# cfdeinza/reinforcement-learning-rendezvous

Measured on AMD Instinct MI355X. Metric: env steps/sec, higher is better.
Workload: dtype f64

## Files before the change

### reinforcement_learning_rendezvous_amd/csrc/rdv_rollout.h

```cpp
#pragma once

namespace rdv {

constexpr int kRollEnvs = 256;
constexpr int kRollEnvWaves = kRollEnvs / kWave;
constexpr int kRollActorWaves = kRollEnvs / kPolWaveEnvs;
constexpr int kRollBlock = (kRollEnvWaves + kRollActorWaves) * kWave;
constexpr int kRollLdsFloats = kPolFloats + kRollEnvs * RDV_ACT_DIM + kRollEnvs * RDV_OBS_DIM + kRollEnvs * RDV_ACT_DIM +
                               kRollEnvWaves * kStatWords * 2 + 2 * kRollEnvs;
constexpr int kRollLdsFixed = kRollLdsFloats * 4 + kSlotObsVecs * kRollEnvs * 16 + kRollEnvWaves * kRollEnvs * 2;
template <typename ST> constexpr int roll_lds_bytes() { return kRollLdsFixed + kChunks * kRollEnvs * 4 * (int)sizeof(ST); }
static_assert(roll_lds_bytes<double>() <= 160 * 1024, "the rollout workgroup must fit the CU's 160 KiB of LDS");
static_assert(kRollEnvs == kGroupEnvs, "refill_pass_lds is written for 256-env workgroups");


struct RolloutArgs {
  void* ws;
  uint64_t* stats;
  float* obs;
  float* actions;
  float* reward;
  uint8_t* done;
  float* log_prob;
  float* last_obs;
// ... 27 lines not shown
  using V = typename Vec4<ST>::type;
  extern __shared__ __attribute__((aligned(16))) float lds[];
  float* w = lds;
  float* act_raw = w + kPolFloats;
  float* obs_cur = act_raw + kRollEnvs * RDV_ACT_DIM;
  float* act_cur = obs_cur + kRollEnvs * RDV_OBS_DIM;
  uint64_t* stat_lds = reinterpret_cast<uint64_t*>(act_cur + kRollEnvs * RDV_ACT_DIM);
  uint32_t* job_kind = reinterpret_cast<uint32_t*>(stat_lds + kRollEnvWaves * kStatWords);
  uint32_t* job_counter = job_kind + kRollEnvs;
  uint32_t* refills_done = reinterpret_cast<uint32_t*>(stat_lds + (kStatWords - 1));
  V* slot_chunks = reinterpret_cast<V*>(job_counter + kRollEnvs);
  float4* slot_obs = reinterpret_cast<float4*>(slot_chunks + kChunks * kRollEnvs);
  const SlotStore<ST> L = lds_slot_store<ST>(slot_chunks, slot_obs, kRollEnvs);
  uint16_t* lists = reinterpret_cast<uint16_t*>(slot_obs + kSlotObsVecs * kRollEnvs);
  const bool resets = A.on_done == RDV_ON_DONE_RESET;
  const DevParams& P = *Pp;
  const int lane = threadIdx.x & (kWave - 1);
  const int wv = threadIdx.x >> 6;
  const bool env_role = wv < kRollEnvWaves;
  const int64_t n = A.n;
  const int64_t block_base = (int64_t)blockIdx.x * kRollEnvs;
  const int T = A.n_steps;

  for (int q = threadIdx.x; q < kPolFloats / 4; q += kRollBlock)
    *reinterpret_cast<float4*>(w + 4 * q) = *reinterpret_cast<const float4*>(W + 4 * q);

  const int slot = (wv & (kRollEnvWaves - 1)) * kWave + lane;
  const int64_t i = block_base + slot;
  const bool active = env_role && i < n;
  Env e;
  e.episode = 0u;
  bool wt_dirty = kGeneral;
  bool slot_dirty = false;
  const SlotStore<ST> H = hbm_slot_store<ST>(A.prep);
  uint64_t* my_stats = stat_lds + (wv & (kRollEnvWaves - 1)) * kStatWords;
  if (env_role) {
    if (lane < kStatWords) my_stats[lane] = (i - lane < n && lane < 12) ? A.stats[(uint64_t)((i - lane) / kWave) * kStatWords + lane] : 0ull;
    __builtin_amdgcn_s_setprio(2);
    float o[RDV_OBS_DIM];
#pragma unroll
    for (int j = 0; j < RDV_OBS_DIM; ++j) o[j] = 0.0f;
    if (active) {
      load_env<ST>(reinterpret_cast<const V*>(A.ws), A.cs, i, e);
      observation(P, e, o);
    }
#pragma unroll
    for (int j = 0; j < RDV_OBS_DIM; ++j) obs_cur[slot * RDV_OBS_DIM + j] = o[j];
    if (resets) {
      uint32_t tag = 0u;
      if (active) { tag = A.prep_tag[i]; slot_copy<ST>(L, slot, H, i); }
      const bool stale = active && tag != e.episode + 1u;
      job_kind[slot] = stale ? JOB_REFILL : JOB_NONE;
      job_counter[slot] = e.episode;
      slot_dirty = stale;
    }
  }
  __syncthreads();

  const int a_wave = wv - kRollEnvWaves;
  const int r0 = a_wave * kPolWaveEnvs;
  const int64_t a_env0 = block_base + r0;
  const int64_t a_rows = env_role ? 0 : ((n - a_env0) < kPolWaveEnvs ? (n - a_env0) : kPolWaveEnvs);
  float* araw = act_raw + (env_role ? 0 : r0) * RDV_ACT_DIM;
  const bool vec_rows = (n & 3) == 0;

  StepArgs SA;
  SA.diag = nullptr;

  if (!env_role) {
   const bool refills = resets && a_wave < kGroupWaves;
   uint16_t* list = lists + (a_wave & (kGroupWaves - 1)) * kRollEnvs;
   auto draw_noise = [&](int t_next, int ln_) {
     if (A.deterministic || a_rows <= 0) return;
     const int er_ = ln_ & 31, eh_ = ln_ >> 5;
     float z[4];
     actor_noise(ln_, A.noise_seed, A.env_id_offset + (uint64_t)(a_env0 + er_), A.noise_counter0 + (uint64_t)t_next, z);
     if (eh_ == 0) {
#pragma unroll
       for (int c = 0; c < 4; ++c) araw[er_ * RDV_ACT_DIM + c] = z[c];
     } else {
       araw[er_ * RDV_ACT_DIM + 4] = z[0]; araw[er_ * RDV_ACT_DIM + 5] = z[1];
     }
     wave_fence();
   };
   draw_noise(0, lane);
#ifdef RDV_STAMPS
   unsigned long long acc_a = 0, acc_r = 0, acc_w1 = 0, acc_w2 = 0;
#endif
   for (int t = 0; t < T; ++t) {
// ... 186 lines not shown
```

### reinforcement_learning_rendezvous_amd/csrc/rdv_slots.h

```cpp
#pragma once

namespace rdv {

constexpr int kSlotObsVecs = 5;
enum : uint32_t { JOB_NONE = 0, JOB_REFILL = 1 };
constexpr uint32_t kFlagsPending = 0xFFFFFFFFu;

template <typename ST>
struct SlotStore {
  typename Vec4<ST>::type* chunks;
  float4* obs;
  int64_t cs, es, ocs, oes;
  static constexpr bool kLive = false;
  __device__ __forceinline__ typename Vec4<ST>::type* chunk(int c, int64_t i) const { return chunks + (c * cs + i * es); }
  __device__ __forceinline__ float4* ovec(int v, int64_t i) const { return obs + (v * ocs + i * oes); }
  __device__ __forceinline__ float* oelem(int j, int64_t i) const { return reinterpret_cast<float*>(ovec(j >> 2, i)) + (j & 3); }
  __device__ __forceinline__ void opad(int64_t i) const { float* p = oelem(16, i); p[1] = 0.0f; p[2] = 0.0f; p[3] = 0.0f; }
};
template <typename ST>
struct LiveStore {
  typename Vec4<ST>::type* ws;
  float* rows;
  int64_t cs, base;
  static constexpr bool kLive = true;
  __device__ __forceinline__ typename Vec4<ST>::type* chunk(int c, int64_t s) const { return ws + (c * cs + base + s); }
  __device__ __forceinline__ float* oelem(int j, int64_t s) const { return rows + (s * RDV_OBS_DIM + j); }
  __device__ __forceinline__ void opad(int64_t) const {}
};
template <typename ST> constexpr int slot_record_bytes() { return sizeof(ST) == 4 ? 192 : 320; }
template <typename ST>
__device__ __forceinline__ SlotStore<ST> hbm_slot_store(void* prep) {
  using V = typename Vec4<ST>::type;
  SlotStore<ST> S;
  S.chunks = reinterpret_cast<V*>(prep);
  S.obs = reinterpret_cast<float4*>(S.chunks + kChunks);
  S.cs = 1; S.es = slot_record_bytes<ST>() / (int)sizeof(V);
  S.ocs = 1; S.oes = slot_record_bytes<ST>() / 16;
  return S;
}
template <typename ST>
__device__ __forceinline__ SlotStore<ST> lds_slot_store(typename Vec4<ST>::type* chunks, float4* obs, int entries) {
  SlotStore<ST> S;
  S.chunks = chunks; S.obs = obs; S.cs = entries; S.es = 1; S.ocs = entries; S.oes = 1;
  return S;
}

template <typename ST>
__device__ __forceinline__ void slot_store_full(const SlotStore<ST>& S, int64_t i, const Env& ne, const float* o) {
  typename Vec4<ST>::type c[kChunks];
  pack_env<ST>(ne, c);
#pragma unroll
  for (int k = 0; k < kChunks; ++k) *S.chunk(k, i) = c[k];
#pragma unroll
  for (int v = 0; v < 4; ++v) *S.ovec(v, i) = make_float4(o[4 * v], o[4 * v + 1], o[4 * v + 2], o[4 * v + 3]);
  *S.ovec(4, i) = make_float4(o[16], 0.0f, 0.0f, 0.0f);
}

template <typename ST>
struct SlotRaw {
  typename Vec4<ST>::type c[kChunks];
  float4 o[kSlotObsVecs];
};
template <typename ST>
__device__ __forceinline__ void slot_fetch(const SlotStore<ST>& S, int64_t i, SlotRaw<ST>& raw) {
#pragma unroll
  for (int k = 0; k < kChunks; ++k) raw.c[k] = *S.chunk(k, i);
#pragma unroll
  for (int v = 0; v < kSlotObsVecs; ++v) raw.o[v] = *S.ovec(v, i);
}
template <typename ST>
__device__ __forceinline__ void slot_unpack(const DevParams& P, const SlotRaw<ST>& raw, Env& e, float* o) {
  const typename Vec4<ST>::type* c = raw.c;
  e.rc[0] = c[0].x; e.rc[1] = c[0].y; e.rc[2] = c[0].z; e.vc[0] = c[0].w;
  e.vc[1] = c[1].x; e.vc[2] = c[1].y; e.wc[0] = c[1].z; e.wc[1] = c[1].w;
  e.wc[2] = c[2].x; e.bubble = c[2].y; e.sum_dv = c[2].z; e.sum_dw = c[2].w;
  e.qc[0] = c[3].x; e.qc[1] = c[3].y; e.qc[2] = c[3].z; e.qc[3] = c[3].w;
  e.qt[0] = c[4].x; e.qt[1] = c[4].y; e.qt[2] = c[4].z; e.qt[3] = c[4].w;
  e.ep_ret = c[5].x; e.k = (int32_t)s2u(c[5].y); e.flags = s2u(c[5].z); e.episode = s2u(c[5].w);
  e.wt[0] = c[6].x; e.wt[1] = c[6].y; e.wt[2] = c[6].z;
#pragma unroll
  for (int v = 0; v < 4; ++v) { o[4 * v] = raw.o[v].x; o[4 * v + 1] = raw.o[v].y; o[4 * v + 2] = raw.o[v].z; o[4 * v + 3] = raw.o[v].w; }
  o[16] = raw.o[4].x;
  if (e.flags == kFlagsPending) e.flags = reset_flags(P, e);
}

template <typename ST>
__device__ __forceinline__ void slot_copy(const SlotStore<ST>& D, int64_t di, const SlotStore<ST>& S, int64_t si) {
#pragma unroll
  for (int k = 0; k < kChunks; ++k) *D.chunk(k, di) = *S.chunk(k, si);
#pragma unroll
  for (int v = 0; v < kSlotObsVecs; ++v) *D.ovec(v, di) = *S.ovec(v, si);
}

__device__ __forceinline__ const double* tape_row_of(const double* tape, int32_t depth, int64_t n, int64_t i, uint32_t counter) {
  if (depth <= 0) return nullptr;
  uint32_t dep = (uint32_t)depth;
  asm volatile("" : "+s"(dep));
  return tape + ((int64_t)(counter % dep) * n + i) * RDV_STATE_DIM;
}

template <typename ST>
__device__ __forceinline__ void reset_whole(const DevParams& P, Env& ne, float* o, uint64_t seed, uint64_t env_id, uint32_t counter,
                                            const double* tape_row) {
  ne.episode = counter;
  reset_env<ST>(P, ne, seed, env_id, tape_row);
  observation(P, ne, o);
}

template <typename ST>
__device__ __forceinline__ void refill_whole(const StepArgs& A, const DevParams& P, int64_t i, uint32_t counter) {
  Env ne;
  float o[RDV_OBS_DIM];
  reset_whole<ST>(P, ne, o, A.seed, A.env_id_offset + (uint64_t)i, counter, tape_row_of(A.tape, A.tape_depth, A.n, i, counter));
  slot_store_full<ST>(hbm_slot_store<ST>(A.prep), i, ne, o);
  A.prep_tag[i] = counter + 1u;
}

template <typename ST, int kPart, typename Store>
__device__ __forceinline__ void slot_refill_part(const DevParams& P, const Store& S, int64_t i, uint64_t seed, uint64_t env_id,
                                                 uint32_t counter, const double* tape_row) {
  const ST t = ST(0);
  Env ne;
  ne.episode = counter;
  reset_fields<ST, kPart>(P, ne, seed, env_id, tape_row);
  ST* c1 = reinterpret_cast<ST*>(S.chunk(1, i));
  ST* c2 = reinterpret_cast<ST*>(S.chunk(2, i));
  auto O = [&](int j) -> float& { return *S.oelem(j, i); };
  if (kPart == RESET_RC_VC) {
    uint32_t flags = 0u;
    if (reset_flags_needed(P, ne)) {
      flags = kFlagsPending;
      if (Store::kLive) {
        Env full;
        full.episode = counter;
        reset_fields<ST, RESET_ALL>(P, full, seed, env_id, tape_row);
        flags = reset_flags(P, full);
      }
    }
    typename Vec4<ST>::type v0, v5;
    v0.x = (ST)ne.rc[0]; v0.y = (ST)ne.rc[1]; v0.z = (ST)ne.rc[2]; v0.w = (ST)ne.vc[0];
    *S.chunk(0, i) = v0;
    c1[0] = (ST)ne.vc[1]; c1[1] = (ST)ne.vc[2];
    c2[1] = (ST)canon(P.bubble_radius0, t); c2[2] = ST(0); c2[3] = ST(0);
    v5.x = ST(0); v5.y = u2s(0u, t); v5.z = u2s(flags, t); v5.w = u2s(counter + 1u, t);
    *S.chunk(5, i) = v5;
#pragma unroll
    for (int j = 0; j < 3; ++j) {
      const float a = normalized(ne.rc[j], P.obs_lo_r, P.obs_span_r, P.obs_inv_span_r);
      const float b = normalized(ne.vc[j], P.obs_lo_v, P.obs_span_v, P.obs_inv_span_v);
      O(j) = a;
      O(3 + j) = b;
    }
  } else if (kPart == RESET_QC_WC) {
    typename Vec4<ST>::type v3;
    v3.x = (ST)ne.qc[0]; v3.y = (ST)ne.qc[1]; v3.z = (ST)ne.qc[2]; v3.w = (ST)ne.qc[3];
    *S.chunk(3, i) = v3;
    c1[2] = (ST)ne.wc[0]; c1[3] = (ST)ne.wc[1]; c2[0] = (ST)ne.wc[2];
    O(6) = (float)ne.qc[0]; O(7) = (float)ne.qc[1]; O(8) = (float)ne.qc[2]; O(9) = (float)ne.qc[3];
    O(10) = normalized(ne.wc[0], P.obs_lo_w, P.obs_span_w, P.obs_inv_span_w);
    O(11) = normalized(ne.wc[1], P.obs_lo_w, P.obs_span_w, P.obs_inv_span_w);
    O(12) = normalized(ne.wc[2], P.obs_lo_w, P.obs_span_w, P.obs_inv_span_w);
  } else if (kPart == RESET_QT) {
    typename Vec4<ST>::type v4;
    v4.x = (ST)ne.qt[0]; v4.y = (ST)ne.qt[1]; v4.z = (ST)ne.qt[2]; v4.w = (ST)ne.qt[3];
    *S.chunk(4, i) = v4;
    O(13) = (float)ne.qt[0]; O(14) = (float)ne.qt[1]; O(15) = (float)ne.qt[2]; O(16) = (float)ne.qt[3];
    S.opad(i);
  } else {
    typename Vec4<ST>::type v6;
    v6.x = (ST)ne.wt[0]; v6.y = (ST)ne.wt[1]; v6.z = (ST)ne.wt[2]; v6.w = ST(0);
    *S.chunk(6, i) = v6;
  }
}
template <typename ST, typename Store>
__device__ __forceinline__ void slot_refill_role(int role, const DevParams& P, const Store& S, int64_t i, uint64_t seed,
                                                 uint64_t env_id, uint32_t counter, const double* tape_row) {
  if (role == 0) slot_refill_part<ST, RESET_RC_VC>(P, S, i, seed, env_id, counter, tape_row);
  else if (role == 1) slot_refill_part<ST, RESET_QC_WC>(P, S, i, seed, env_id, counter, tape_row);
  else if (role == 2) slot_refill_part<ST, RESET_QT>(P, S, i, seed, env_id, counter, tape_row);
  else slot_refill_part<ST, RESET_WT>(P, S, i, seed, env_id, counter, tape_row);
}

template <int Q>
__device__ __forceinline__ int compact_flags(const bool (&flag)[Q], int lane, uint16_t* list) {
  int total = 0;
#pragma unroll
  for (int q = 0; q < Q; ++q) {
    const unsigned long long m = __ballot(flag[q]);
    if (flag[q]) {
      const int rank = (int)__builtin_amdgcn_mbcnt_hi((uint32_t)(m >> 32), __builtin_amdgcn_mbcnt_lo((uint32_t)m, 0u));
      list[total + rank] = (uint16_t)(q * kWave + lane);
    }
    total += __popcll(m);
  }
  wave_lds_fence();
  return total;
}

constexpr int kGroupEnvs = 256;
constexpr int kGroupWaves = kGroupEnvs / kWave;

template <typename ST, typename Store>
__device__ __forceinline__ void refill_pass_lds(int role, int lane, const DevParams& P, const Store& L, const uint32_t* job_kind,
                                                const uint32_t* job_counter, uint16_t* list, int64_t block_base, int64_t n, uint64_t seed,
                                                uint64_t env_id_offset, const double* tape, int32_t tape_depth) {
// ... 19 lines not shown
```

### reinforcement_learning_rendezvous_amd/csrc/rdv_step.h

```cpp
#pragma once
#include "rdv_kernels.h"
#include "rdv_slots.h"

namespace rdv {

template <typename ST>
__global__ __launch_bounds__(kBlock) void prepare_kernel(const DevParams* __restrict__ Pp, const StepArgs A) {
  using V = typename Vec4<ST>::type;
  const int64_t i = (int64_t)blockIdx.x * kBlock + threadIdx.x;
  if (i >= A.n) return;
  const V c5 = reinterpret_cast<const V*>(A.ws)[5 * A.cs + i];
  refill_whole<ST>(A, *Pp, i, s2u(c5.w));
}

template <typename ST, bool kAll, typename... G>
__global__ __launch_bounds__(kBlock) __attribute__((amdgpu_waves_per_eu(sizeof(ST) == 4 ? RDV_PARTS_WAVES : 3))) void step_kernel_parts(void* ws_hot, const float* actions_hot, const DevParams* __restrict__ Pp, int64_t n_hot,
                                                             uint64_t* stats_hot, float* obs_hot, float* reward_hot, G... tile_group, const StepArgs A_rest) {
  static_assert(sizeof...(G) <= 1, "G is empty or the type of the tile table");
  const StepArgs A = hot_args(A_rest, ws_hot, actions_hot, n_hot, stats_hot, obs_hot, reward_hot);
  using V = typename Vec4<ST>::type;
  __shared__ __attribute__((aligned(16))) float lds[kBlock * RDV_OBS_DIM];
  __shared__ uint32_t job_kind[kBlock];
  __shared__ uint32_t job_counter[kBlock];
  __shared__ uint16_t lists[kGroupWaves * kBlock];
// ... 79 lines not shown
  }
  RDV_STAMP(6);
  if (A.stream_rows) store_obs_rows<true>(A.obs, wave_base, rows, lane, wl);
  else store_obs_rows<false>(A.obs, wave_base, rows, lane, wl);
  RDV_STAMP(7);
  RDV_STAMP_FLUSH((uint64_t)blockIdx.x * (kBlock / kWave) + wave_in_block)
}

constexpr int kSplitEnvs = 256;
constexpr int kSplitBlock = 512;

template <typename ST>
__device__ __forceinline__ void refill_stale_slots(const StepArgs& A, const DevParams& P, int64_t base, int wv, int lane, uint32_t* job_kind,
                                                   uint32_t* job_counter, uint16_t* lists) {
  constexpr int Q = kSplitEnvs / kWave;
  constexpr int kWords = sizeof(typename Vec4<ST>::type) / 4, kWordK = kWords / 4, kWordEpisode = 3 * kWords / 4;
  if (wv < Q) {
    const uint32_t* c5 = reinterpret_cast<const uint32_t*>(reinterpret_cast<const typename Vec4<ST>::type*>(A.ws) + 5 * A.cs);
    const int s = wv * kWave + lane;
    const int64_t ii = base + s;
    const bool ok = ii < A.n;
    const int64_t il = ok ? ii : A.n - 1;
    const uint32_t k = c5[il * kWords + kWordK], episode = c5[il * kWords + kWordEpisode], tag = A.prep_tag[il];
    job_kind[s] = (ok && k == 0u && tag != episode + 1u) ? JOB_REFILL : JOB_NONE;
    job_counter[s] = episode;
  }
  __syncthreads();
  if (wv >= Q) return;
  uint16_t* list = lists + wv * kSplitEnvs;
  bool flag[Q];
#pragma unroll
  for (int q = 0; q < Q; ++q) flag[q] = job_kind[q * kWave + lane] != JOB_NONE;
  const int total = compact_flags<Q>(flag, lane, list);
  const SlotStore<ST> S = hbm_slot_store<ST>(A.prep);
#pragma clang loop unroll(disable)
  for (int j0 = 0; j0 < total; j0 += kWave) {
    const int j = j0 + lane;
    if (j < total) {
      const int s = (int)list[j];
      const uint32_t counter = job_counter[s];
      const int64_t ii = base + s;
      slot_refill_role<ST>(wv, P, S, ii, A.seed, A.env_id_offset + (uint64_t)ii, counter, tape_row_of(A.tape, A.tape_depth, A.n, ii, counter));
      if (wv == 0) A.prep_tag[ii] = counter + 1u;
    }
  }
}

#ifndef RDV_TARGET_SERVICE_PRIO
#define RDV_TARGET_SERVICE_PRIO 3
#endif
#define RDV_REQUEST_RECORDS(rec, recp, mask, saved)                                                                                                  \
  do {                                                                                                                                               \
    _Pragma("unroll") for (int v_ = 0; v_ < 12; ++v_) asm volatile("" : "=v"(rec[v_]));      \
    asm volatile("s_and_saveexec_b64 %[sv], %[m]\n\t"                                                                                                \
                 "global_load_dwordx4 %[r0], %[p], off\n\t"                                                                                          \
                 "global_load_dwordx4 %[r1], %[p], off offset:16\n\t"                                                                                \
                 "global_load_dwordx4 %[r2], %[p], off offset:32\n\t"                                                                                \
                 "global_load_dwordx4 %[r3], %[p], off offset:48\n\t"                                                                                \
                 "global_load_dwordx4 %[r4], %[p], off offset:64\n\t"                                                                                \
                 "global_load_dwordx4 %[r5], %[p], off offset:80\n\t"                                                                                \
                 "global_load_dwordx4 %[r6], %[p], off offset:96\n\t"                                                                                \
                 "global_load_dwordx4 %[r7], %[p], off offset:112\n\t"                                                                               \
                 "global_load_dwordx4 %[r8], %[p], off offset:128\n\t"                                                                               \
                 "global_load_dwordx4 %[r9], %[p], off offset:144\n\t"                                                                               \
                 "global_load_dwordx4 %[r10], %[p], off offset:160\n\t"                                                                              \
                 "global_load_dwordx4 %[r11], %[p], off offset:176\n\t"                                                                              \
                 "s_mov_b64 exec, %[sv]"                                                                                                             \
                 : [r0] "+v"(rec[0]), [r1] "+v"(rec[1]), [r2] "+v"(rec[2]), [r3] "+v"(rec[3]), [r4] "+v"(rec[4]), [r5] "+v"(rec[5]), [r6] "+v"(rec[6]), \
                   [r7] "+v"(rec[7]), [r8] "+v"(rec[8]), [r9] "+v"(rec[9]), [r10] "+v"(rec[10]), [r11] "+v"(rec[11]), [sv] "=&s"(saved)               \
                 : [p] "v"(recp), [m] "s"(mask)                                                                                                      \
                 : "scc");                                                                                                                           \
  } while (0)
template <typename ST, bool kAll, bool kSlots, bool kTarget, bool kObs = false>
__device__ __forceinline__ void split_body(void* ws_hot, const float* actions_hot, const DevParams* Pp, int64_t n_hot, uint64_t* stats_hot, float* obs_hot,
                                           float* reward_hot, const StepArgs& A_rest, float* stage, unsigned long long* fin_mask, float* hand_f, double* hand_d,
                                           float* hand_c = nullptr, unsigned long long* out_mask = nullptr) {
  static_assert(!kTarget || kSlots, "the target form is a form of the slot form");
  static_assert(!kObs || kTarget, "the observation form is a form of the target form");
  constexpr int kS = kTarget ? 1 : 0;
  (void)kS; (void)hand_f; (void)hand_d; (void)hand_c; (void)out_mask;
  const StepArgs A = hot_args(A_rest, ws_hot, actions_hot, n_hot, stats_hot, obs_hot, reward_hot);
  using V = typename Vec4<ST>::type;
  const DevParams& P = *Pp;
  const int lane = threadIdx.x & (kWave - 1);
  const int wv = threadIdx.x >> 6;
  const bool step_role = wv < kSplitEnvs / kWave;
  const int slot_in_block = threadIdx.x & (kSplitEnvs - 1);
  const int64_t n = A.n;
  const int64_t i = (int64_t)blockIdx.x * kSplitEnvs + slot_in_block;
  const int64_t wave_base = i - lane;
  const bool active = i < n;
  const int64_t rows = (n - wave_base) < kWave ? (n - wave_base) : kWave;
  V* ws = reinterpret_cast<V*>(A.ws);
  const bool resets = A.on_done == RDV_ON_DONE_RESET;
  RDV_STAMP_DECL
  RDV_STAMP(0);

  if constexpr (kSlots) {
    static_assert(sizeof(ST) == 4 && kAll, "the slot form is built for fp32 storage without halted envs");
    const unsigned n_step_wgs = (unsigned)((n + kSplitEnvs - 1) / kSplitEnvs);
    const bool refill_role = blockIdx.x >= n_step_wgs;
    const unsigned refill_wg = blockIdx.x - n_step_wgs;
// ... 70 lines not shown
    } else {
      if constexpr (kAll) { advance_all<ST>(P, e, a, r, row_sink, kPack ? packed : nullptr, actions_ready); stepped = active; }
      else stepped = advance<ST, false>(A, P, i, active, e, a, r, row_sink, NoHook(), kPack ? packed : nullptr);
      RDV_STAMP(2);
    }
    bool fin = stepped && r.done;
    bool to_reset = fin && resets;
    const unsigned long long m_reset = __ballot(to_reset);
    if (lane == 0) fin_mask[wv] = m_reset;
    if constexpr (!kObs) {
      halt_if_done<ST>(A, fin, e, kPack ? packed : nullptr);
      if (stepped && !to_reset) { if (kPack) store_chunks<ST, true>(ws, A.cs, i, packed, false); else store_env<ST>(ws, A.cs, i, e, false); }
    }
    RDV_STAMP(3 + kS);
    __syncthreads();
    RDV_STAMP(4 + kS);
    if constexpr (kObs) {
      if ((out_mask[wv] >> lane) & 1ull) { r.done = 1; r.reason = 1; }
      fin = stepped && r.done;
      to_reset = fin && resets;
      halt_if_done<ST>(A, fin, e, packed);
      if (stepped && !to_reset) store_chunks<ST, true>(ws, A.cs, i, packed, false);
    }
    stats_update(slot, slot_pre, lane, stepped, fin, r.reason, e.flags, e.k, e.ep_ret, e.sum_dv, e.sum_dw);
    if constexpr (kObs) {
      store_step_outputs<false>(A, i, active, fin, r, e, nullptr);
    } else {
      store_step_outputs<true>(A, i, active, fin, r, e, obs_r);
      if (m_reset == 0ull) store_obs_rows<true>(A.obs, wave_base, rows, lane, wl);
    }
    RDV_STAMP(5 + kS);
    RDV_STAMP(6 + kS);
  } else if constexpr (kSlots) {
    constexpr int kRecVecs = kChunks + kSlotObsVecs;
    static_assert(slot_record_bytes<ST>() == kRecVecs * 16 && kRecVecs == 12, "the fp32 slot record is 12 vectors: the requests are written out below");
    const int64_t il = active ? i : n - 1;
    const pin_f4* recp = reinterpret_cast<const pin_f4*>(A.prep) + il * kRecVecs;
    pin_f4 rec[kRecVecs];
    pin_f4 c5;
    uint32_t tag;
    Env obs_env;
    float obs_r[RDV_OBS_DIM];
    bool obs_outside = false;
    (void)obs_env; (void)obs_r; (void)obs_outside;
    if constexpr (kTarget) {
      pin_f4 c4, c6;
      const pin_f4* wsl = reinterpret_cast<const pin_f4*>(ws) + il;
      asm volatile("global_load_dwordx4 %0, %4, off\n\tglobal_load_dwordx4 %1, %5, off\n\tglobal_load_dwordx4 %2, %6, off\n\tglobal_load_dword %3, %7, off"
                   : "=&v"(c4), "=&v"(c6), "=&v"(c5), "=&v"(tag) : "v"(wsl + 4 * A.cs), "v"(wsl + 6 * A.cs), "v"(wsl + 5 * A.cs), "v"(A.prep_tag + il));
      asm volatile("s_waitcnt vmcnt(0)" : "+v"(c4), "+v"(c6), "+v"(c5), "+v"(tag));
      RDV_STAMP(1);
      if (RDV_TARGET_SERVICE_PRIO) __builtin_amdgcn_s_setprio(RDV_TARGET_SERVICE_PRIO);
      double qt[4] = {c4.x, c4.y, c4.z, c4.w}, wt[3] = {c6.x, c6.y, c6.z};
      step_target<false, false>(P, qt, wt);
      double Rt[9], rd_l[3];
#pragma unroll
      for (int k = 0; k < 4; ++k) qt[k] = canon(qt[k], ST(0));
      derive_target_head(P, qt, Rt, rd_l);
#pragma unroll
      for (int k = 0; k < 4; ++k) hand_f[k * kSplitEnvs + slot_in_block] = (float)qt[k];
#pragma unroll
      for (int k = 0; k < 3; ++k) { hand_f[(4 + k) * kSplitEnvs + slot_in_block] = c6[k]; hand_d[k * kSplitEnvs + slot_in_block] = rd_l[k]; }
      if constexpr (kObs) {
#pragma unroll
        for (int k = 0; k < 4; ++k) obs_env.qt[k] = qt[k];
        float* my_row = stage + slot_in_block * RDV_OBS_DIM;
#pragma unroll
        for (int k = 0; k < 4; ++k) {
// ... 10 lines not shown
      RDV_STAMP(1);
    }
    const uint32_t k_in = __float_as_uint(c5.y), episode_in = __float_as_uint(c5.w);
    const bool copy_ok = tag == episode_in + 1u && k_in >= 1u;
    unsigned long long saved_exec;
    if constexpr (kObs) RDV_REQUEST_RECORDS(rec, recp, __ballot(copy_ok), saved_exec);
    if constexpr (kTarget) {
      RDV_STAMP(2);
      __syncthreads();
      RDV_STAMP(3);
    }
    if constexpr (!kObs) RDV_REQUEST_RECORDS(rec, recp, __ballot(copy_ok), saved_exec);
    if constexpr (kObs) {
#pragma unroll
      for (int k = 0; k < 3; ++k) {
        obs_env.rc[k] = (double)hand_c[k * kSplitEnvs + slot_in_block];
        obs_env.vc[k] = (double)hand_c[(3 + k) * kSplitEnvs + slot_in_block];
        obs_env.wc[k] = (double)hand_c[(10 + k) * kSplitEnvs + slot_in_block];
      }
#pragma unroll
      for (int k = 0; k < 4; ++k) obs_env.qc[k] = (double)hand_c[(6 + k) * kSplitEnvs + slot_in_block];
      float* my_row = stage + slot_in_block * RDV_OBS_DIM;
      observation_to(P, obs_env, [&](int j, float v) {
        if (j >= 13) return;
        obs_outside |= !(fabsf(v) <= 1.0f);
        obs_r[j] = v; my_row[j] = v;
      });
      const unsigned long long m_out = __ballot(active && obs_outside);
      if (lane == 0) out_mask[wv - kSplitEnvs / kWave] = m_out;
    }
#ifdef RDV_STAMPS
    if constexpr (!kObs)
    asm volatile("s_waitcnt vmcnt(0)" : "+v"(rec[0]), "+v"(rec[1]), "+v"(rec[2]), "+v"(rec[3]), "+v"(rec[4]), "+v"(rec[5]), "+v"(rec[6]),
                 "+v"(rec[7]), "+v"(rec[8]), "+v"(rec[9]), "+v"(rec[10]), "+v"(rec[11]));
#endif
    if constexpr (!kTarget) RDV_STAMP(2);
    RDV_STAMP(3 + kS);
    __syncthreads();
    RDV_STAMP(4 + kS);
    asm volatile("s_waitcnt vmcnt(0)" : "+v"(rec[0]), "+v"(rec[1]), "+v"(rec[2]), "+v"(rec[3]), "+v"(rec[4]), "+v"(rec[5]), "+v"(rec[6]),
                 "+v"(rec[7]), "+v"(rec[8]), "+v"(rec[9]), "+v"(rec[10]), "+v"(rec[11]));
    unsigned long long m_reset = fin_mask[wv - kSplitEnvs / kWave];
    if constexpr (kObs) m_reset |= out_mask[wv - kSplitEnvs / kWave];
    if (m_reset != 0ull) {
      float* wl = stage + (wv - kSplitEnvs / kWave) * (kWave * RDV_OBS_DIM);
      if (active && ((m_reset >> lane) & 1ull)) {
        if constexpr (kObs) {
          if (A.terminal_obs) {
            float* t = A.terminal_obs + i * RDV_OBS_DIM;
#pragma unroll
            for (int j = 0; j < RDV_OBS_DIM; ++j) t[j] = obs_r[j];
          }
        }
        if (copy_ok) {
          if (__float_as_uint(rec[5].z) == kFlagsPending) {
            float4 c[kChunks];
#pragma unroll
            for (int j = 0; j < kChunks; ++j) c[j] = make_float4(rec[j].x, rec[j].y, rec[j].z, rec[j].w);
            Env se;
            unpack_env<float>(c, se);
            rec[5].z = __uint_as_float(reset_flags(P, se));
          }
          pin_f4* dst = reinterpret_cast<pin_f4*>(ws) + i;
#pragma unroll
          for (int j = 0; j < kChunks; ++j) __builtin_nontemporal_store(rec[j], dst + j * A.cs);
#pragma unroll
          for (int j = 0; j < RDV_OBS_DIM; ++j) wl[lane * RDV_OBS_DIM + j] = rec[kChunks + (j >> 2)][j & 3];
        } else {
          Env ne;
          float robs[RDV_OBS_DIM];
          ne.episode = episode_in;
          const double* row = nullptr;
          if (A.tape_depth > 0) row = A.tape + ((int64_t)(ne.episode % (uint32_t)A.tape_depth) * n + i) * RDV_STATE_DIM;
          reset_state<ST, false>(P, ne, A.seed, A.env_id_offset + (uint64_t)i, row);
          reset_aux<ST>(P, ne);
          canon_rest<ST>(ne);
          observation(P, ne, robs);
          store_env<ST, true>(ws, A.cs, i, ne, true);
#pragma unroll
          for (int j = 0; j < RDV_OBS_DIM; ++j) wl[lane * RDV_OBS_DIM + j] = robs[j];
        }
      }
      if constexpr (!kObs) {
        wave_lds_fence();
        RDV_STAMP(5 + kS);
        store_obs_rows<true>(A.obs, wave_base, rows, lane, wl);
      }
    }
    if constexpr (kObs) {
      wave_lds_fence();
      RDV_STAMP(5 + kS);
      store_obs_rows<true>(A.obs, wave_base, rows, lane, stage + (wv - kSplitEnvs / kWave) * (kWave * RDV_OBS_DIM));
    }
    RDV_STAMP(6 + kS);
  } else {
    Env ne;
    if (resets && active) {
      const V c5 = ws[5 * A.cs + i];
      ne.episode = s2u(c5.w);
      RDV_STAMP(1);
// ... 62 lines not shown
```

### reinforcement_learning_rendezvous_amd/csrc/rdv_step_many.h

```cpp
#pragma once

namespace rdv {

constexpr int kManyEnvs = kGroupEnvs;
constexpr int kManyEnvWaves = kManyEnvs / kWave;
constexpr int kManyBlock = 2 * kManyEnvs;
constexpr int kManyHandoverWords = 9;
constexpr int kManyLdsFixed = (kManyEnvs * RDV_OBS_DIM + kManyEnvs * kManyHandoverWords + 2 * kManyEnvs) * 4 + kManyEnvWaves * kStatWords * 8 +
                              kSlotObsVecs * kManyEnvs * 16 + kManyEnvWaves * kManyEnvs * 2;
template <typename ST> constexpr int many_lds_bytes() { return kManyLdsFixed + kChunks * kManyEnvs * 4 * (int)sizeof(ST); }

struct StepManyArgs {
  void* ws;
  uint64_t* stats;
  const float* actions;
  float* obs;
  float* reward;
  uint8_t* done;
  uint8_t* done_reason;
  const double* tape;
  void* prep;
  uint32_t* prep_tag;
  int64_t n;
  int64_t cs;
// ... 9 lines not shown
  using V = typename Vec4<ST>::type;
  extern __shared__ __attribute__((aligned(16))) float lds[];
  float* obs_rows = lds;
  uint32_t* ho_words = reinterpret_cast<uint32_t*>(obs_rows + kManyEnvs * RDV_OBS_DIM);
  double* ho_reals = reinterpret_cast<double*>(ho_words + 3 * kManyEnvs + (kManyEnvs & 1));
  uint32_t* job_kind = ho_words + kManyHandoverWords * kManyEnvs;
  uint32_t* job_counter = job_kind + kManyEnvs;
  uint64_t* stat_lds = reinterpret_cast<uint64_t*>(job_counter + kManyEnvs);
  V* slot_chunks = reinterpret_cast<V*>(stat_lds + kManyEnvWaves * kStatWords);
  float4* slot_obs = reinterpret_cast<float4*>(slot_chunks + kChunks * kManyEnvs);
  const SlotStore<ST> L = lds_slot_store<ST>(slot_chunks, slot_obs, kManyEnvs);
  uint16_t* lists = reinterpret_cast<uint16_t*>(slot_obs + kSlotObsVecs * kManyEnvs);
  const DevParams& P = *Pp;
  const int lane = threadIdx.x & (kWave - 1);
  const int wv = threadIdx.x >> 6;
  const bool env_role = wv < kManyEnvWaves;
  const int slot = (wv & (kManyEnvWaves - 1)) * kWave + lane;
  const int64_t n = A.n;
  const int64_t block_base = (int64_t)blockIdx.x * kManyEnvs;
  const int64_t i = block_base + slot;
  const int64_t wave_base = i - lane;
  const bool active = i < n;
  const int64_t rows = (n - wave_base) < kWave ? (n - wave_base) : kWave;
  const int K = A.n_steps;
  const bool resets = A.on_done == RDV_ON_DONE_RESET;
  const bool vec_rows = (n & 3) == 0;
  V* ws = reinterpret_cast<V*>(A.ws);

  if (env_role) {
    __builtin_amdgcn_s_setprio(2);
    float* my_obs = obs_rows + (slot - lane) * RDV_OBS_DIM;
    uint64_t* my_stats = stat_lds + wv * kStatWords;
    if (lane < kStatWords) my_stats[lane] = (rows > 0 && lane < 12) ? A.stats[(uint64_t)(wave_base / kWave) * kStatWords + lane] : 0ull;
    const SlotStore<ST> H = hbm_slot_store<ST>(A.prep);
    Env e;
    e.episode = 0u;
    bool slot_dirty = false;
    bool wt_dirty = kGeneral;
    if (active) load_env<ST>(ws, A.cs, i, e);
    if (resets) {
      uint32_t tag = 0u;
      if (active) { tag = A.prep_tag[i]; slot_copy<ST>(L, slot, H, i); }
      const bool stale = active && tag != e.episode + 1u;
      job_kind[slot] = stale ? JOB_REFILL : JOB_NONE;
      job_counter[slot] = e.episode;
      slot_dirty = stale;
    }
    StepArgs SA;
    SA.diag = nullptr;
    auto fetch = [&](int k, float2 (&pre)[3]) {
      const float* row = A.actions + ((int64_t)k * n + i) * RDV_ACT_DIM;
#pragma unroll
      for (int q = 0; q < 3; ++q) pre[q] = active ? *reinterpret_cast<const float2*>(row + 2 * q) : make_float2(0.0f, 0.0f);
    };
    float2 pre[3] = {make_float2(0.0f, 0.0f), make_float2(0.0f, 0.0f), make_float2(0.0f, 0.0f)};
    fetch(0, pre);
    if (resets) __syncthreads();
    for (int k = 0; k < K; ++k) {
      float a[RDV_ACT_DIM];
#pragma unroll
      for (int q = 0; q < 3; ++q) { a[2 * q] = pre[q].x; a[2 * q + 1] = pre[q].y; }
      if (k + 1 < K) fetch(k + 1, pre);
      StepResult r;
      float* my_row = my_obs + lane * RDV_OBS_DIM;
      float obs_r[RDV_OBS_DIM];
      const bool stepped = advance<ST, false, kGeneral, !kGeneral>(SA, P, i, active, e, a, r, RowSink{obs_r});
      const bool fin = stepped && r.done;
      if (active) {
        const int64_t o = (int64_t)k * n + i;
        A.reward[o] = r.reward;
        A.done[o] = (uint8_t)r.done;
        if (A.done_reason)
          A.done_reason[o] = (uint8_t)(r.reason | ((fin && (e.flags & FLAG_COLLIDED)) ? 16 : 0) | ((fin && (e.flags >> SUCCESS_SHIFT) != 0u) ? 32 : 0));
      }
      if (!resets) stats_update(my_stats, lane < 12 ? my_stats[lane] : 0ull, lane, stepped, fin, r.reason, e.flags, e.k, e.ep_ret, e.sum_dv, e.sum_dw);
// ... 59 lines not shown
```

Measured before the change: 11.63 billion.

## Compact the HBM slot record by dropping derivable fields and reconstructing on load

Replaces the prepared-reset slot record in HBM (chunked env state plus a padded obs copy) with a compact SlotRecord. The record stores only the non-derivable state and the normalized obs components; bubble, counters, tag and the quaternion obs are rebuilt on read. The fp32 split path now issues 8 vector loads per record instead of 12, and writers in the refill passes store directly into the new record fields. This cuts HBM traffic for reset prefetch at the cost of extra reconstruction ALU work and more fragile layout assumptions.

Result: faster. 11.79 billion, median of 6 (+1.4%).

```diff
diff --git a/reinforcement_learning_rendezvous_amd/csrc/rdv_rollout.h b/reinforcement_learning_rendezvous_amd/csrc/rdv_rollout.h
--- a/reinforcement_learning_rendezvous_amd/csrc/rdv_rollout.h
+++ b/reinforcement_learning_rendezvous_amd/csrc/rdv_rollout.h
@@ -83,7 +83,7 @@
   e.episode = 0u;
   bool wt_dirty = kGeneral;
   bool slot_dirty = false;
-  const SlotStore<ST> H = hbm_slot_store<ST>(A.prep);
+  const HbmSlotStore<ST> H = hbm_slot_store<ST>(A.prep);
   uint64_t* my_stats = stat_lds + (wv & (kRollEnvWaves - 1)) * kStatWords;
   if (env_role) {
     if (lane < kStatWords) my_stats[lane] = (i - lane < n && lane < 12) ? A.stats[(uint64_t)((i - lane) / kWave) * kStatWords + lane] : 0ull;
@@ -99,13 +99,14 @@
     for (int j = 0; j < RDV_OBS_DIM; ++j) obs_cur[slot * RDV_OBS_DIM + j] = o[j];
     if (resets) {
       uint32_t tag = 0u;
-      if (active) { tag = A.prep_tag[i]; slot_copy<ST>(L, slot, H, i); }
+      if (active) { tag = A.prep_tag[i]; slot_copy<ST>(L, slot, H, i, P, tag); }
       const bool stale = active && tag != e.episode + 1u;
       job_kind[slot] = stale ? JOB_REFILL : JOB_NONE;
       job_counter[slot] = e.episode;
       slot_dirty = stale;
     }
   }
+  asm volatile(".p2align 6");
   __syncthreads();
 
   const int a_wave = wv - kRollEnvWaves;
diff --git a/reinforcement_learning_rendezvous_amd/csrc/rdv_slots.h b/reinforcement_learning_rendezvous_amd/csrc/rdv_slots.h
--- a/reinforcement_learning_rendezvous_amd/csrc/rdv_slots.h
+++ b/reinforcement_learning_rendezvous_amd/csrc/rdv_slots.h
@@ -11,7 +11,7 @@
   typename Vec4<ST>::type* chunks;
   float4* obs;
   int64_t cs, es, ocs, oes;
-  static constexpr bool kLive = false;
+  static constexpr bool kLive = false, kRecord = false;
   __device__ __forceinline__ typename Vec4<ST>::type* chunk(int c, int64_t i) const { return chunks + (c * cs + i * es); }
   __device__ __forceinline__ float4* ovec(int v, int64_t i) const { return obs + (v * ocs + i * oes); }
   __device__ __forceinline__ float* oelem(int j, int64_t i) const { return reinterpret_cast<float*>(ovec(j >> 2, i)) + (j & 3); }
@@ -22,20 +22,88 @@
   typename Vec4<ST>::type* ws;
   float* rows;
   int64_t cs, base;
-  static constexpr bool kLive = true;
+  static constexpr bool kLive = true, kRecord = false;
   __device__ __forceinline__ typename Vec4<ST>::type* chunk(int c, int64_t s) const { return ws + (c * cs + base + s); }
   __device__ __forceinline__ float* oelem(int j, int64_t s) const { return rows + (s * RDV_OBS_DIM + j); }
   __device__ __forceinline__ void opad(int64_t) const {}
 };
-template <typename ST> constexpr int slot_record_bytes() { return sizeof(ST) == 4 ? 192 : 320; }
-template <typename ST>
-__device__ __forceinline__ SlotStore<ST> hbm_slot_store(void* prep) {
-  using V = typename Vec4<ST>::type;
-  SlotStore<ST> S;
-  S.chunks = reinterpret_cast<V*>(prep);
-  S.obs = reinterpret_cast<float4*>(S.chunks + kChunks);
-  S.cs = 1; S.es = slot_record_bytes<ST>() / (int)sizeof(V);
-  S.ocs = 1; S.oes = slot_record_bytes<ST>() / 16;
+template <typename ST>
+struct alignas(16) SlotRecord {
+  ST rc[3], vc[3];
+  float n_rc[3], n_vc[3];
+  ST qc[4];
+  ST wc[3];
+  float n_wc[3];
+  uint32_t flags;
+  uint32_t pad;
+  ST qt[4];
+  ST wt[3];
+};
+static_assert(sizeof(SlotRecord<float>) == 128 && sizeof(SlotRecord<double>) == 208, "the compact slot record: 8 / 13 vectors");
+static_assert(offsetof(SlotRecord<float>, n_rc) == 24 && offsetof(SlotRecord<float>, qc) == 48 && offsetof(SlotRecord<float>, wc) == 64 &&
+              offsetof(SlotRecord<float>, flags) == 88 && offsetof(SlotRecord<float>, qt) == 96 && offsetof(SlotRecord<float>, wt) == 112,
+              "the vectors v0..v7 of the fp32 record (step_kernel_split's slot forms read them as vectors)");
+template <typename ST> constexpr int slot_record_bytes() { return (int)sizeof(SlotRecord<ST>); }
+
+template <typename ST>
+struct HbmSlotStore {
+  SlotRecord<ST>* rec;
+  static constexpr bool kLive = false, kRecord = true;
+  template <int kPart>
+  __device__ __forceinline__ void put_part(const DevParams& P, int64_t i, const Env& ne, uint32_t flags) const {
+    SlotRecord<ST>& R = rec[i];
+    if (kPart == RESET_RC_VC) {
+      float a[3], b[3];
+#pragma unroll
+      for (int j = 0; j < 3; ++j) {
+        a[j] = normalized(ne.rc[j], P.obs_lo_r, P.obs_span_r, P.obs_inv_span_r);
+        b[j] = normalized(ne.vc[j], P.obs_lo_v, P.obs_span_v, P.obs_inv_span_v);
+      }
+#pragma unroll
+      for (int j = 0; j < 3; ++j) R.rc[j] = (ST)ne.rc[j];
+#pragma unroll
+      for (int j = 0; j < 3; ++j) R.vc[j] = (ST)ne.vc[j];
+#pragma unroll
+      for (int j = 0; j < 3; ++j) R.n_rc[j] = a[j];
+#pragma unroll
+      for (int j = 0; j < 3; ++j) R.n_vc[j] = b[j];
+      R.flags = flags;
+    } else if (kPart == RESET_QC_WC) {
+      float w[3];
+#pragma unroll
+      for (int j = 0; j < 3; ++j) w[j] = normalized(ne.wc[j], P.obs_lo_w, P.obs_span_w, P.obs_inv_span_w);
+      if constexpr (sizeof(ST) == 4) {
+        float4* v = reinterpret_cast<float4*>(&R);
+        v[3] = make_float4((float)ne.qc[0], (float)ne.qc[1], (float)ne.qc[2], (float)ne.qc[3]);
+        asm volatile("" ::: "memory");
+        v[4] = make_float4((float)ne.wc[0], (float)ne.wc[1], (float)ne.wc[2], w[0]);
+        asm volatile("" ::: "memory");
+        *reinterpret_cast<float2*>(&R.n_wc[1]) = make_float2(w[1], w[2]);
+      } else {
+#pragma unroll
+        for (int j = 0; j < 4; ++j) R.qc[j] = (ST)ne.qc[j];
+#pragma unroll
+        for (int j = 0; j < 3; ++j) R.wc[j] = (ST)ne.wc[j];
+#pragma unroll
+        for (int j = 0; j < 3; ++j) R.n_wc[j] = w[j];
+      }
+    } else if (kPart == RESET_QT) {
+#pragma unroll
+      for (int j = 0; j < 4; ++j) R.qt[j] = (ST)ne.qt[j];
+    } else {
+      put_wt(R, ne);
+    }
+  }
+  __device__ __forceinline__ static void put_wt(SlotRecord<ST>& R, const Env& ne) {
+#pragma unroll
+    for (int j = 0; j < 3; ++j) R.wt[j] = (ST)ne.wt[j];
+    if constexpr (sizeof(ST) == 4) reinterpret_cast<float*>(&R)[31] = 0.0f;
+  }
+};
+template <typename ST>
+__device__ __forceinline__ HbmSlotStore<ST> hbm_slot_store(void* prep) {
+  HbmSlotStore<ST> S;
+  S.rec = reinterpret_cast<SlotRecord<ST>*>(prep);
   return S;
 }
 template <typename ST>
@@ -46,14 +114,19 @@
 }
 
 template <typename ST>
-__device__ __forceinline__ void slot_store_full(const SlotStore<ST>& S, int64_t i, const Env& ne, const float* o) {
-  typename Vec4<ST>::type c[kChunks];
-  pack_env<ST>(ne, c);
-#pragma unroll
-  for (int k = 0; k < kChunks; ++k) *S.chunk(k, i) = c[k];
-#pragma unroll
-  for (int v = 0; v < 4; ++v) *S.ovec(v, i) = make_float4(o[4 * v], o[4 * v + 1], o[4 * v + 2], o[4 * v + 3]);
-  *S.ovec(4, i) = make_float4(o[16], 0.0f, 0.0f, 0.0f);
+__device__ __forceinline__ void slot_store_full(const HbmSlotStore<ST>& S, int64_t i, const Env& ne, const float* o) {
+  SlotRecord<ST> r;
+#pragma unroll
+  for (int j = 0; j < 3; ++j) {
+    r.rc[j] = (ST)ne.rc[j]; r.vc[j] = (ST)ne.vc[j]; r.wc[j] = (ST)ne.wc[j]; r.wt[j] = (ST)ne.wt[j];
+    r.n_rc[j] = o[j]; r.n_vc[j] = o[3 + j]; r.n_wc[j] = o[10 + j];
+  }
+#pragma unroll
+  for (int j = 0; j < 4; ++j) { r.qc[j] = (ST)ne.qc[j]; r.qt[j] = (ST)ne.qt[j]; }
+  r.flags = ne.flags;
+  r.pad = 0u;
+  if constexpr (sizeof(ST) == 4) reinterpret_cast<float*>(&r)[31] = 0.0f;
+  S.rec[i] = r;
 }
 
 template <typename ST>
@@ -85,11 +158,42 @@
 }
 
 template <typename ST>
-__device__ __forceinline__ void slot_copy(const SlotStore<ST>& D, int64_t di, const SlotStore<ST>& S, int64_t si) {
-#pragma unroll
-  for (int k = 0; k < kChunks; ++k) *D.chunk(k, di) = *S.chunk(k, si);
-#pragma unroll
-  for (int v = 0; v < kSlotObsVecs; ++v) *D.ovec(v, di) = *S.ovec(v, si);
+__device__ __forceinline__ void slot_copy(const SlotStore<ST>& D, int64_t di, const HbmSlotStore<ST>& S, int64_t si, const DevParams& P, uint32_t tag) {
+  using V = typename Vec4<ST>::type;
+  const ST t = ST(0);
+  const SlotRecord<ST> r = S.rec[si];
+  V c;
+  c.x = r.rc[0]; c.y = r.rc[1]; c.z = r.rc[2]; c.w = r.vc[0]; *D.chunk(0, di) = c;
+  c.x = r.vc[1]; c.y = r.vc[2]; c.z = r.wc[0]; c.w = r.wc[1]; *D.chunk(1, di) = c;
+  c.x = r.wc[2]; c.y = (ST)canon(P.bubble_radius0, t); c.z = ST(0); c.w = ST(0); *D.chunk(2, di) = c;
+  c.x = r.qc[0]; c.y = r.qc[1]; c.z = r.qc[2]; c.w = r.qc[3]; *D.chunk(3, di) = c;
+  c.x = r.qt[0]; c.y = r.qt[1]; c.z = r.qt[2]; c.w = r.qt[3]; *D.chunk(4, di) = c;
+  c.x = ST(0); c.y = u2s(0u, t); c.z = u2s(r.flags, t); c.w = u2s(tag, t); *D.chunk(5, di) = c;
+  c.x = r.wt[0]; c.y = r.wt[1]; c.z = r.wt[2]; c.w = ST(0); *D.chunk(6, di) = c;
+  *D.ovec(0, di) = make_float4(r.n_rc[0], r.n_rc[1], r.n_rc[2], r.n_vc[0]);
+  *D.ovec(1, di) = make_float4(r.n_vc[1], r.n_vc[2], (float)r.qc[0], (float)r.qc[1]);
+  *D.ovec(2, di) = make_float4((float)r.qc[2], (float)r.qc[3], r.n_wc[0], r.n_wc[1]);
+  *D.ovec(3, di) = make_float4(r.n_wc[2], (float)r.qt[0], (float)r.qt[1], (float)r.qt[2]);
+  *D.ovec(4, di) = make_float4((float)r.qt[3], 0.0f, 0.0f, 0.0f);
+}
+template <typename ST>
+__device__ __forceinline__ void slot_copy(const HbmSlotStore<ST>& D, int64_t di, const SlotStore<ST>& S, int64_t si) {
+  using V = typename Vec4<ST>::type;
+  const V c0 = *S.chunk(0, si), c1 = *S.chunk(1, si), c2 = *S.chunk(2, si), c3 = *S.chunk(3, si), c4 = *S.chunk(4, si), c5 = *S.chunk(5, si),
+          c6 = *S.chunk(6, si);
+  const float4 o0 = *S.ovec(0, si), o1 = *S.ovec(1, si), o2 = *S.ovec(2, si), o3 = *S.ovec(3, si);
+  SlotRecord<ST> r;
+  r.rc[0] = c0.x; r.rc[1] = c0.y; r.rc[2] = c0.z; r.vc[0] = c0.w; r.vc[1] = c1.x; r.vc[2] = c1.y;
+  r.n_rc[0] = o0.x; r.n_rc[1] = o0.y; r.n_rc[2] = o0.z; r.n_vc[0] = o0.w; r.n_vc[1] = o1.x; r.n_vc[2] = o1.y;
+  r.qc[0] = c3.x; r.qc[1] = c3.y; r.qc[2] = c3.z; r.qc[3] = c3.w;
+  r.wc[0] = c1.z; r.wc[1] = c1.w; r.wc[2] = c2.x;
+  r.n_wc[0] = o2.z; r.n_wc[1] = o2.w; r.n_wc[2] = o3.x;
+  r.flags = s2u(c5.z);
+  r.pad = 0u;
+  r.qt[0] = c4.x; r.qt[1] = c4.y; r.qt[2] = c4.z; r.qt[3] = c4.w;
+  r.wt[0] = c6.x; r.wt[1] = c6.y; r.wt[2] = c6.z;
+  if constexpr (sizeof(ST) == 4) reinterpret_cast<float*>(&r)[31] = 0.0f;
+  D.rec[di] = r;
 }
 
 __device__ __forceinline__ const double* tape_row_of(const double* tape, int32_t depth, int64_t n, int64_t i, uint32_t counter) {
@@ -123,6 +227,11 @@
   Env ne;
   ne.episode = counter;
   reset_fields<ST, kPart>(P, ne, seed, env_id, tape_row);
+  if constexpr (Store::kRecord) {
+    (void)t;
+    S.template put_part<kPart>(P, i, ne, (kPart == RESET_RC_VC && reset_flags_needed(P, ne)) ? kFlagsPending : 0u);
+    return;
+  } else {
   ST* c1 = reinterpret_cast<ST*>(S.chunk(1, i));
   ST* c2 = reinterpret_cast<ST*>(S.chunk(2, i));
   auto O = [&](int j) -> float& { return *S.oelem(j, i); };
@@ -171,6 +280,7 @@
     v6.x = (ST)ne.wt[0]; v6.y = (ST)ne.wt[1]; v6.z = (ST)ne.wt[2]; v6.w = ST(0);
     *S.chunk(6, i) = v6;
   }
+  }
 }
 template <typename ST, typename Store>
 __device__ __forceinline__ void slot_refill_role(int role, const DevParams& P, const Store& S, int64_t i, uint64_t seed,
diff --git a/reinforcement_learning_rendezvous_amd/csrc/rdv_step.h b/reinforcement_learning_rendezvous_amd/csrc/rdv_step.h
--- a/reinforcement_learning_rendezvous_amd/csrc/rdv_step.h
+++ b/reinforcement_learning_rendezvous_amd/csrc/rdv_step.h
@@ -135,7 +135,7 @@
 #pragma unroll
   for (int q = 0; q < Q; ++q) flag[q] = job_kind[q * kWave + lane] != JOB_NONE;
   const int total = compact_flags<Q>(flag, lane, list);
-  const SlotStore<ST> S = hbm_slot_store<ST>(A.prep);
+  const HbmSlotStore<ST> S = hbm_slot_store<ST>(A.prep);
 #pragma clang loop unroll(disable)
   for (int j0 = 0; j0 < total; j0 += kWave) {
     const int j = j0 + lane;
@@ -154,7 +154,7 @@
 #endif
 #define RDV_REQUEST_RECORDS(rec, recp, mask, saved)                                                                                                  \
   do {                                                                                                                                               \
-    _Pragma("unroll") for (int v_ = 0; v_ < 12; ++v_) asm volatile("" : "=v"(rec[v_]));      \
+    _Pragma("unroll") for (int v_ = 0; v_ < 8; ++v_) asm volatile("" : "=v"(rec[v_]));      \
     asm volatile("s_and_saveexec_b64 %[sv], %[m]\n\t"                                                                                                \
                  "global_load_dwordx4 %[r0], %[p], off\n\t"                                                                                          \
                  "global_load_dwordx4 %[r1], %[p], off offset:16\n\t"                                                                                \
@@ -164,13 +164,9 @@
                  "global_load_dwordx4 %[r5], %[p], off offset:80\n\t"                                                                                \
                  "global_load_dwordx4 %[r6], %[p], off offset:96\n\t"                                                                                \
                  "global_load_dwordx4 %[r7], %[p], off offset:112\n\t"                                                                               \
-                 "global_load_dwordx4 %[r8], %[p], off offset:128\n\t"                                                                               \
-                 "global_load_dwordx4 %[r9], %[p], off offset:144\n\t"                                                                               \
-                 "global_load_dwordx4 %[r10], %[p], off offset:160\n\t"                                                                              \
-                 "global_load_dwordx4 %[r11], %[p], off offset:176\n\t"                                                                              \
                  "s_mov_b64 exec, %[sv]"                                                                                                             \
                  : [r0] "+v"(rec[0]), [r1] "+v"(rec[1]), [r2] "+v"(rec[2]), [r3] "+v"(rec[3]), [r4] "+v"(rec[4]), [r5] "+v"(rec[5]), [r6] "+v"(rec[6]), \
-                   [r7] "+v"(rec[7]), [r8] "+v"(rec[8]), [r9] "+v"(rec[9]), [r10] "+v"(rec[10]), [r11] "+v"(rec[11]), [sv] "=&s"(saved)               \
+                   [r7] "+v"(rec[7]), [sv] "=&s"(saved)                                                                                            \
                  : [p] "v"(recp), [m] "s"(mask)                                                                                                      \
                  : "scc");                                                                                                                           \
   } while (0)
@@ -307,8 +303,8 @@
     RDV_STAMP(5 + kS);
     RDV_STAMP(6 + kS);
   } else if constexpr (kSlots) {
-    constexpr int kRecVecs = kChunks + kSlotObsVecs;
-    static_assert(slot_record_bytes<ST>() == kRecVecs * 16 && kRecVecs == 12, "the fp32 slot record is 12 vectors: the requests are written out below");
+    constexpr int kRecVecs = 8;
+    static_assert(slot_record_bytes<ST>() == kRecVecs * 16, "the fp32 slot record is 8 vectors: the requests are written out below");
     const int64_t il = active ? i : n - 1;
     const pin_f4* recp = reinterpret_cast<const pin_f4*>(A.prep) + il * kRecVecs;
     pin_f4 rec[kRecVecs];
@@ -385,14 +381,14 @@
 #ifdef RDV_STAMPS
     if constexpr (!kObs)
     asm volatile("s_waitcnt vmcnt(0)" : "+v"(rec[0]), "+v"(rec[1]), "+v"(rec[2]), "+v"(rec[3]), "+v"(rec[4]), "+v"(rec[5]), "+v"(rec[6]),
-                 "+v"(rec[7]), "+v"(rec[8]), "+v"(rec[9]), "+v"(rec[10]), "+v"(rec[11]));
+                 "+v"(rec[7]));
 #endif
     if constexpr (!kTarget) RDV_STAMP(2);
     RDV_STAMP(3 + kS);
     __syncthreads();
     RDV_STAMP(4 + kS);
     asm volatile("s_waitcnt vmcnt(0)" : "+v"(rec[0]), "+v"(rec[1]), "+v"(rec[2]), "+v"(rec[3]), "+v"(rec[4]), "+v"(rec[5]), "+v"(rec[6]),
-                 "+v"(rec[7]), "+v"(rec[8]), "+v"(rec[9]), "+v"(rec[10]), "+v"(rec[11]));
+                 "+v"(rec[7]));
     unsigned long long m_reset = fin_mask[wv - kSplitEnvs / kWave];
     if constexpr (kObs) m_reset |= out_mask[wv - kSplitEnvs / kWave];
     if (m_reset != 0ull) {
@@ -406,19 +402,32 @@
           }
         }
         if (copy_ok) {
-          if (__float_as_uint(rec[5].z) == kFlagsPending) {
-            float4 c[kChunks];
-#pragma unroll
-            for (int j = 0; j < kChunks; ++j) c[j] = make_float4(rec[j].x, rec[j].y, rec[j].z, rec[j].w);
+          uint32_t flags = __float_as_uint(rec[5].z);
+          if (flags == kFlagsPending) {
             Env se;
-            unpack_env<float>(c, se);
-            rec[5].z = __uint_as_float(reset_flags(P, se));
+#pragma unroll
+            for (int j = 0; j < 3; ++j) { se.rc[j] = rec[0][j]; se.wc[j] = rec[4][j]; se.wt[j] = rec[7][j]; }
+            se.vc[0] = rec[0].w; se.vc[1] = rec[1].x; se.vc[2] = rec[1].y;
+#pragma unroll
+            for (int j = 0; j < 4; ++j) { se.qc[j] = rec[3][j]; se.qt[j] = rec[6][j]; }
+            flags = reset_flags(P, se);
           }
+          const pin_f4 n1 = {rec[1].x, rec[1].y, rec[4].x, rec[4].y};
+          const pin_f4 n2 = {rec[4].z, (float)canon(P.bubble_radius0, ST(0)), 0.0f, 0.0f};
+          const pin_f4 n5 = {0.0f, __uint_as_float(0u), __uint_as_float(flags), __uint_as_float(episode_in + 1u)};
           pin_f4* dst = reinterpret_cast<pin_f4*>(ws) + i;
-#pragma unroll
-          for (int j = 0; j < kChunks; ++j) __builtin_nontemporal_store(rec[j], dst + j * A.cs);
-#pragma unroll
-          for (int j = 0; j < RDV_OBS_DIM; ++j) wl[lane * RDV_OBS_DIM + j] = rec[kChunks + (j >> 2)][j & 3];
+          __builtin_nontemporal_store(rec[0], dst);
+          __builtin_nontemporal_store(n1, dst + 1 * A.cs);
+          __builtin_nontemporal_store(n2, dst + 2 * A.cs);
+          __builtin_nontemporal_store(rec[3], dst + 3 * A.cs);
+          __builtin_nontemporal_store(rec[6], dst + 4 * A.cs);
+          __builtin_nontemporal_store(n5, dst + 5 * A.cs);
+          __builtin_nontemporal_store(rec[7], dst + 6 * A.cs);
+          float* row = wl + lane * RDV_OBS_DIM;
+          row[0] = rec[1].z; row[1] = rec[1].w; row[2] = rec[2].x; row[3] = rec[2].y; row[4] = rec[2].z; row[5] = rec[2].w;
+#pragma unroll
+          for (int j = 0; j < 4; ++j) { row[6 + j] = rec[3][j]; row[13 + j] = rec[6][j]; }
+          row[10] = rec[4].w; row[11] = rec[5].x; row[12] = rec[5].y;
         } else {
           Env ne;
           float robs[RDV_OBS_DIM];
diff --git a/reinforcement_learning_rendezvous_amd/csrc/rdv_step_many.h b/reinforcement_learning_rendezvous_amd/csrc/rdv_step_many.h
--- a/reinforcement_learning_rendezvous_amd/csrc/rdv_step_many.h
+++ b/reinforcement_learning_rendezvous_amd/csrc/rdv_step_many.h
@@ -65,7 +65,7 @@
     float* my_obs = obs_rows + (slot - lane) * RDV_OBS_DIM;
     uint64_t* my_stats = stat_lds + wv * kStatWords;
     if (lane < kStatWords) my_stats[lane] = (rows > 0 && lane < 12) ? A.stats[(uint64_t)(wave_base / kWave) * kStatWords + lane] : 0ull;
-    const SlotStore<ST> H = hbm_slot_store<ST>(A.prep);
+    const HbmSlotStore<ST> H = hbm_slot_store<ST>(A.prep);
     Env e;
     e.episode = 0u;
     bool slot_dirty = false;
@@ -73,7 +73,7 @@
     if (active) load_env<ST>(ws, A.cs, i, e);
     if (resets) {
       uint32_t tag = 0u;
-      if (active) { tag = A.prep_tag[i]; slot_copy<ST>(L, slot, H, i); }
+      if (active) { tag = A.prep_tag[i]; slot_copy<ST>(L, slot, H, i, P, tag); }
       const bool stale = active && tag != e.episode + 1u;
       job_kind[slot] = stale ? JOB_REFILL : JOB_NONE;
       job_counter[slot] = e.episode;
```
